# Alisah-Ozcan/GPU-NTT

Hardware: AMD Instinct MI355X
Metric: forward-NTTs/sec + achieved HBM GB/s, 64-bit Merge N=2^16 batch=1024 (higher is better)
Workload: dtype u64; 1 GPU; Merge-NTT Data64 log2N=16 batch=1024 forward (BASELINE configs[1]); log2N=16, batch_per_gpu=1024, reduction_poly=X_N_minus, modulus=576460756061519873, in_place=True, api=dropin, parallelism=batch-shard x1

## Files before the change

### gpu-ntt_amd/csrc/launch.hpp

```cpp
#pragma once

#include <hip/hip_runtime.h>

#include <stdexcept>

#include "gpuntt/common/common.cuh"
#include "merge_kernels.hpp"

#ifndef GPUNTT_SHADOW_GRID
#define GPUNTT_SHADOW_GRID 512
#endif

namespace gpuntt
{
    namespace host
    {
        void note_launch(const char* kernel_expr, int family = -1);
    }
}
#define GPUNTT_LAUNCH(kernel, ...)                                                                                       \
    do                                                                                                                   \
    {                                                                                                                    \
        ::gpuntt::host::note_launch(#kernel);                                                                            \
        hipLaunchKernelGGL(kernel, __VA_ARGS__);                                                                         \
    } while (0)
#define GPUNTT_LAUNCH_FAMILY(family, kernel, ...)                                                                        \
    do                                                                                                                   \
    {                                                                                                                    \
        ::gpuntt::host::note_launch(#kernel, family);                                                                    \
        hipLaunchKernelGGL(kernel, __VA_ARGS__);                                                                         \
    } while (0)

namespace gpuntt
{
    namespace host
    {
        struct Pass
        {
            bool contig;
            int k;
            int p_lo;
            int in_b = 0;
            bool p4 = false;
        };

        struct Plan
        {
            Pass pass[8];
            int count;
        };

        inline Plan make_plan(int n, int contig_k = kern::TL)
        {
            Plan pl{};
            pl.count = 0;
            if (n <= kern::TL)
            {
                pl.pass[pl.count++] = Pass{true, n, 0};
                return pl;
            }
            if (contig_k > kern::TL)
                contig_k = kern::TL;
            if (contig_k < 8)
                contig_k = 8;
            const int s = n - contig_k;
            const int np = (s + 7) / 8;
            int top = n;
            for (int i = 0; i < np; i++)
            {
                const int k = s / np + ((i < s % np) ? 1 : 0);
                top -= k;
                pl.pass[pl.count++] = Pass{false, k, top};
            }
            pl.pass[pl.count++] = Pass{true, contig_k, 0};
            return pl;
// ... 39 lines not shown
```

### gpu-ntt_amd/csrc/lazy.hpp

```cpp
#pragma once

#include <hip/hip_runtime.h>

#include <cstdint>

namespace gpuntt
{
    namespace lazy
    {
        template <typename T> struct Tw;
        template <> struct alignas(16) Tw<uint64_t>
        {
            uint64_t w;
            uint64_t wp;
        };
        template <> struct alignas(8) Tw<uint32_t>
        {
            uint32_t w;
            uint32_t wp;
        };
        using Tw64 = Tw<uint64_t>;
        using Tw32 = Tw<uint32_t>;

        __device__ __forceinline__ uint32_t lo32(uint64_t v) { return static_cast<uint32_t>(v); }
// ... 51 lines not shown
            uint64_t d, cy;
            if constexpr (SB)
                asm("v_mad_u64_u32 %0, %1, %2, %3, -1" : "=v"(d), "=s"(cy) : "v"(a), "s"(b));
            else
                asm("v_mad_u64_u32 %0, %1, %2, %3, -1" : "=v"(d), "=s"(cy) : "v"(a), "v"(b));
            return d;
        }
        __device__ __forceinline__ uint32_t xad_not(uint32_t w, uint32_t u) { return (w ^ 0xffffffffu) + u; }

        template <int LIM, bool VQ = false> struct Mod64
        {
            static constexpr int TB = (LIM == 4) ? 2 : 4;
            static constexpr int LIMIT = LIM;
            static constexpr int MAX_BIT = (LIM == 16 || LIM == 31) ? 60 : (LIM == 8 ? 61 : 62);
            uint64_t q;
            uint64_t qneg;
            NormConst nc;
            uint32_t zero;
            uint32_t one;

            __device__ __forceinline__ void set(uint64_t modulus, const NormConst& n)
            {
                q = modulus;
                qneg = 0 - modulus;
                nc = n;
                asm("v_mov_b32 %0, 0" : "=v"(zero));
                asm("v_mov_b32 %0, 1" : "=v"(one));
            }
            template <bool HI = false> __device__ __forceinline__ uint64_t reduce_2q(uint64_t x) const
            {
                const uint32_t xt = HI ? hi32(x) : static_cast<uint32_t>(x >> nc.sh);
                const uint32_t k = __umulhi(xt, nc.M) >> nc.c;
                const uint64_t r = static_cast<uint64_t>(k) * lo32(qneg) + x;
                return r + (static_cast<uint64_t>(k * hi32(qneg)) << 32);
            }
            __device__ __forceinline__ uint64_t kq(int k) const { return q * static_cast<uint64_t>(k); }
            __device__ __forceinline__ bool hi_norm() const { return nc.hi != 0u; }

            template <bool UNI, bool ZERO = false>
            __device__ __forceinline__ uint64_t mul_acc(uint64_t x, const Tw64& t, uint64_t acc) const
            {
                if constexpr (LIM == 4)
                {
                    const uint64_t p = csub<2>(mul_acc_raw<UNI, true>(x, t, 0));
                    return ZERO ? p : acc + p;
                }
                else
                    return mul_acc_raw<UNI, ZERO>(x, t, acc);
            }
            template <bool UNI, bool ZERO>
            __device__ __forceinline__ uint64_t mul_acc_raw(uint64_t x, const Tw64& t, uint64_t acc) const
            {
                const uint32_t x0 = lo32(x), x1 = hi32(x);
                const uint32_t h2 = __umulhi(x0, hi32(t.wp));
                uint64_t qh, carry;
                if constexpr (UNI)
                    asm("v_mul_hi_u32 v126, %2, %3\n\tv_mad_u64_u32 %0, %1, %2, %4, v[126:127]"
                        : "=v"(qh), "=s"(carry)
                        : "v"(x1), "s"(lo32(t.wp)), "s"(hi32(t.wp)), "{v127}"(zero)
                        : "v126");
                else
                    asm("v_mul_hi_u32 v126, %2, %3\n\tv_mad_u64_u32 %0, %1, %2, %4, v[126:127]"
                        : "=v"(qh), "=s"(carry)
                        : "v"(x1), "v"(lo32(t.wp)), "v"(hi32(t.wp)), "{v127}"(zero)
                        : "v126");
                qh = static_cast<uint64_t>(h2) * one + qh;
                uint64_t c = static_cast<uint64_t>(x0) * hi32(t.w);
// ... 145 lines not shown
            if constexpr (B > 2)
                x = m.template csub<2>(x);
            if constexpr (B > 1)
                x = m.template csub<1>(x);
            return x;
        }

        constexpr int ceil_pow2(int v)
        {
            int p = 1;
            while (p < v)
                p <<= 1;
            return p;
        }
        constexpr int csub_k(int b) { return ceil_pow2(b) / 2; }

        struct CtPlan
        {
            int ku;
            int out;
        };
        constexpr CtPlan ct_plan(int bu, int limit, int tb)
        {
            CtPlan p{0, 0};
            if (bu + tb > limit)
            {
                p.ku = csub_k(bu);
                bu = p.ku;
            }
            p.out = bu + tb;
            return p;
        }

        struct GsPlan
        {
            int ku, kv;
            int c;
            int ko;
            int out_u;
        };
        constexpr GsPlan gs_plan(int bu, int bv, int limit)
        {
            GsPlan p{0, 0, 0, 0, 0};
            const int half = limit / 2;
            if (bu > half)
            {
                p.ku = csub_k(bu);
                bu = p.ku;
            }
            if (bv > half)
            {
                p.kv = csub_k(bv);
                bv = p.kv;
            }
            p.c = ceil_pow2(bv);
            int out = bu + bv;
            if (out > half)
            {
                p.ko = csub_k(out);
                out = p.ko;
            }
            p.out_u = out;
            return p;
        }
    }
}
// ... 1 lines not shown
```

### gpu-ntt_amd/csrc/lazy_launch.hpp

```cpp
#pragma once

#include <hip/hip_runtime.h>

#include <string>

#include "launch.hpp"
#include "merge_lazy_kernels.hpp"

namespace gpuntt
{
    namespace host
    {
        constexpr int LAZY_MAX_N_POWER = 28;

        constexpr int lazy_u32_tile_override() { return 0; }
        constexpr int lazy_u64_big_tiles() { return 14; }

        bool lazy_two_sweep_big();
        bool lazy_contig_p4();
        void note_contig_p4_launch();
        unsigned long long contig_p4_launches();
        constexpr int LAZY_P4_N_POWER = 16;
        constexpr unsigned long long lazy_u32_small_batch() { return 0x7fffffffull; }
        template <typename T> inline int lazy_tile_log(int n, bool inverse = false, unsigned long long polys = 0)
// ... 320 lines not shown
        extern template void launch_pass_lazy_lim<false, 4>(const Pass&, bool, bool, const kern::LazyArgsT<uint64_t>&, hipStream_t);
        template <bool INV, int LIMSEL>
        void launch_fourstep_lim(int what, int log_n1, const kern::LazyArgsT<uint64_t>& a, hipStream_t stream);
        extern template void launch_fourstep_lim<false, 8>(int, int, const kern::LazyArgsT<uint64_t>&, hipStream_t);
        extern template void launch_fourstep_lim<true, 8>(int, int, const kern::LazyArgsT<uint64_t>&, hipStream_t);
        extern template void launch_fourstep_lim<false, 4>(int, int, const kern::LazyArgsT<uint64_t>&, hipStream_t);
        extern template void launch_fourstep_lim<true, 4>(int, int, const kern::LazyArgsT<uint64_t>&, hipStream_t);
        template <typename TU> inline bool modulus_fast(const Modulus<TU>& m)
        {
            const TU max_bit = (sizeof(TU) == 8) ? TU(62) : TU(lazy::Mod<TU>::MAX_BIT);
            return m.value >= 3 && m.bit <= max_bit;
        }
        template <typename TU> inline int modulus_lim(const Modulus<TU>& m)
        {
            if (sizeof(TU) != 8)
                return 0;
            return m.bit == TU(62) ? 4 : (m.bit == TU(61) ? 8 : 0);
        }
        void launch_pass_lazy31(const Pass& p, int tile_log, bool in_first, bool last, const kern::LazyArgsT<uint64_t>& a,
                                hipStream_t stream);
        constexpr bool lazy_lim31_enabled() { return true; }
        constexpr unsigned lazy_order_flags() { return 0u; }
        template <bool INV>
        void launch_pass_lazy_u32w(const Pass& p, int tile_log, bool in_first, bool last,
                                   const kern::LazyArgsT<uint32_t>& a, hipStream_t stream);
        template <>
        void launch_pass_lazy_u32w<false>(const Pass&, int, bool, bool, const kern::LazyArgsT<uint32_t>&, hipStream_t);
        template <>
        void launch_pass_lazy_u32w<true>(const Pass&, int, bool, bool, const kern::LazyArgsT<uint32_t>&, hipStream_t);
        inline bool lazy_wide_modulus32(uint32_t q) { return q >= 3 && q < (1u << 29); }
        inline bool lazy_lim31_modulus(uint64_t q) { return q >= 3 && q <= 0xffffffffffffffffull / 31; }
        extern template void launch_pass_lazy_lim<true, 4>(const Pass&, bool, bool, const kern::LazyArgsT<uint64_t>&, hipStream_t);

        inline int fwd_bound_after(int bound, int k, int limit, int tb)
        {
            for (int s = 0; s < k; s++)
                bound = lazy::ct_plan(bound, limit, tb).out;
            return bound;
        }

        template <typename T, bool INV>
        inline void run_transform_lazy(kern::LazyArgsT<T> base, unsigned first_in_flags,
                                       unsigned last_out_flags, hipStream_t stream, int forced_tl = 0, int low_stages = 0)
        {
            const int tl = (sizeof(T) == 8 && base.lim && base.lim != 31)
                               ? 12
                               : (forced_tl ? forced_tl : lazy_tile_log_merge<T>(base.n, INV, base.total >> base.n));
            const int pn = (!INV && low_stages > 0) ? low_stages : base.n;
            const bool partial = pn != base.n;
            if constexpr (sizeof(T) == 4)
                if (!partial && base.n == tl && tl >= 12 && tl <= 15 &&
                    (tl == 15 || ((lazy_e32_mask() >> tl) & 1u) != 0u) && (base.total & ((1ull << tl) - 1ull)) == 0ull)
                {
                    kern::LazyArgsT<uint32_t> a = base;
                    a.p_lo = 0;
                    a.flags |= first_in_flags | last_out_flags;
                    return launch_ring_e32<INV>(tl, base.lim, a, stream);
                }
            if (base.mods != nullptr && base.mod_count > 1 && base.n < tl && base.n - kern::R < 6)
            {
                if (base.n < LAZY_MIN_RNS_N_POWER || partial)
                    throw std::invalid_argument("internal: RNS ring too small for the fast path");
                kern::LazyArgsT<T> a = base;
                a.p_lo = 0;
                a.flags |= first_in_flags | last_out_flags;
                return launch_small_rns_lazy<T, INV>(base.n, a, stream);
            }
            const bool big2 = sizeof(T) == 8 && tl == 14 && pn >= 23 && !partial;
            const Plan pl = make_plan_tl(pn, tl, tl == 12 ? (partial ? lazy_contig_k(pn) : lazy_contig_k_merge<T>(pn, INV)) : tl,
                                         big2 ? 10 : (sizeof(T) == 4 && tl == 15) ? 9 : 8);
            const void* src = base.in;
            int fwd_bound = partial ? 16 : 1;
            for (int i = 0; i < pl.count; i++)
            {
                Pass p = INV ? pl.pass[pl.count - 1 - i] : pl.pass[i];
                if (!INV && sizeof(T) == 8 && base.lim == 31)
                {
                    p.in_b = fwd_bound;
                    fwd_bound = fwd_bound_after(fwd_bound, p.k, 31, 4);
                }
                kern::LazyArgsT<T> a = base;
                a.in = src;
                a.p_lo = p.p_lo;
                a.flags |= lazy_order_flags();
                const bool first = (i == 0) && !partial;
                if (i == 0)
                    a.flags |= first_in_flags;
                if (i == pl.count - 1)
                    a.flags |= last_out_flags;
                if (((pl.count - 1 - i) & 1) != 0 && lazy_reverse_passes())
                    a.flags |= kern::F_REVERSE;
                const int tlp = (sizeof(T) == 8 && !p.contig && p.k <= 8) ? 12 : (sizeof(T) == 4 && tl == 15 && !p.contig) ? 14 : tl;
                const unsigned long long polys = base.total >> base.n;
                a.batch = (p.contig && base.n >= 20 && base.n >= tlp && polys >= 2 && polys <= 0x7fffffffull &&
                           (polys << base.n) == base.total)
                              ? static_cast<int>(polys)
                              : 0;
                if constexpr (sizeof(T) == 8 && !INV)
                {
                    const unsigned long long mc = base.mods != nullptr ? static_cast<unsigned long long>(base.mod_count) : 1ull;
                    p.p4 = p.contig && p.k == 10 && tlp == 12 && i == pl.count - 1 && pl.count > 1 && !partial &&
                           base.n == LAZY_P4_N_POWER && base.poly_shift == base.n && mc >= 1 && polys % (4ull * mc) == 0 &&
                           (polys << base.n) == base.total && base.poly_order == nullptr && base.mod_order == nullptr &&
                           base.mul_in == nullptr && a.batch == 0 && lazy_contig_p4();
                }
                if constexpr (sizeof(T) == 4)
                {
                    const bool edge = INV ? (i == 0 && pl.count > 1) : (i == pl.count - 1 && (pl.count > 1 || partial));
                    if (p.contig && p.k == tlp && (tlp == 12 || tlp == 14 || tlp == 15) && edge &&
                        (tlp == 15 || ((lazy_e32_mask() >> 16) & 1u) != 0u))
                    {
                        launch_tile_e32<INV>(tlp, base.lim, a, stream);
                        src = base.out;
                        continue;
                    }
                }
                if constexpr (sizeof(T) == 8)
                {
                    if (base.lim == 8)
                        launch_pass_lazy_lim<INV, 8>(p, first, i == pl.count - 1, a, stream);
                    else if (base.lim == 4)
                        launch_pass_lazy_lim<INV, 4>(p, first, i == pl.count - 1, a, stream);
                    else if (base.lim == 31)
                    {
                        if constexpr (!INV)
// ... 20 lines not shown
```

### gpu-ntt_amd/csrc/lazy_launch_impl.hpp

```cpp
#pragma once

#include "lazy_launch.hpp"

namespace gpuntt
{
    namespace host
    {
        template <typename T, int TLOG, bool INV, bool CONTIG, int K, int IN_BOUND, bool LAST, int LIMSEL = 0, bool P4 = false>
        inline void launch_lazy_one(const kern::LazyArgsT<T>& a, unsigned grid, hipStream_t stream)
        {
            if constexpr (P4)
                note_contig_p4_launch();
            GPUNTT_LAUNCH_FAMILY(LIMSEL, (kern::merge_pass_lazy<T, TLOG, INV, CONTIG, K, IN_BOUND, LAST, LIMSEL, 0, P4>), dim3(grid),
                               dim3(kern::LTile<TLOG>::NT), 0, stream, a);
            GPUNTT_HIP_CHECK(hipGetLastError());
        }

        template <typename T, int TLOG, bool INV, int LIMSEL = 0>
        void dispatch_tl(const Pass& p, bool in_first, bool last, const kern::LazyArgsT<T>& a,
                         hipStream_t stream)
        {
            constexpr int LIM = lazy::Mod<T, LIMSEL>::LIMIT;
            constexpr int TILE = kern::LTile<TLOG>::TILE;
            const unsigned long long tiles = (a.total + TILE - 1) >> TLOG;
            if (tiles == 0)
                return;
            if (tiles > 0x7fffffffull)
                throw std::invalid_argument("batch_size * N too large for one launch");
            const unsigned grid = lazy_grid_cap<T, LIMSEL>(tiles, a.go_flag);
#define GPUNTT_ONE(CONTIG_, K_, IN_, LAST_)                                                      \
    return launch_lazy_one<T, TLOG, INV, CONTIG_, K_, IN_, LAST_, LIMSEL>(a, grid, stream)
            if constexpr (sizeof(T) == 8 && TLOG >= 13)
            {
                if (p.contig && p.k == TLOG)
                {
                    if (in_first && last)
                        GPUNTT_ONE(true, TLOG, 1, true);
                    if constexpr (!INV)
                    {
                        if (!in_first && last)
                            GPUNTT_ONE(true, TLOG, LIM, true);
                    }
                    else
                    {
                        if (in_first && !last)
                            GPUNTT_ONE(true, TLOG, 1, false);
                    }
                }
                if constexpr (TLOG == 14 && !INV)
                    if (!p.contig && in_first && !last)
                    {
                        if (p.k == 9)
                            GPUNTT_ONE(false, 9, 1, false);
                        if (p.k == 10)
                            GPUNTT_ONE(false, 10, 1, false);
                    }
                throw std::invalid_argument("internal: unsupported 64-bit big-tile pass");
            }
            else
            {
            if (p.contig)
            {
// ... 12 lines not shown
                            case 8: GPUNTT_ONE(true, 8, 1, true);
                            case 9: GPUNTT_ONE(true, 9, 1, true);
                            case 10: GPUNTT_ONE(true, 10, 1, true);
                            case 11: GPUNTT_ONE(true, 11, 1, true);
                            case 12: GPUNTT_ONE(true, 12, 1, true);
                            default: break;
                        }
                    else if constexpr (TLOG == 13)
                    {
                        if (p.k == 13)
                            GPUNTT_ONE(true, 13, 1, true);
                    }
                    else
                        switch (p.k)
                        {
                            case 13: GPUNTT_ONE(true, 13, 1, true);
                            case 14: GPUNTT_ONE(true, 14, 1, true);
                            default: break;
                        }
                }
                else if (!INV && !in_first && last)
                {
                    if constexpr (!INV)
                    {
                        if constexpr (TLOG == 12)
                            switch (p.k)
                            {
                                case 8: GPUNTT_ONE(true, 8, LIM, true);
                                case 9: GPUNTT_ONE(true, 9, LIM, true);
                                case 10:
                                    if constexpr (sizeof(T) == 8)
                                        if (p.p4)
                                        {
                                            if constexpr (LIM == 31)
                                                if (p.in_b > 0 && p.in_b <= 27)
                                                    return launch_lazy_one<T, TLOG, INV, true, 10, 27, true, LIMSEL, true>(a, grid, stream);
                                            return launch_lazy_one<T, TLOG, INV, true, 10, LIM, true, LIMSEL, true>(a, grid, stream);
                                        }
                                    if constexpr (LIM == 31)
                                        if (p.in_b > 0 && p.in_b <= 27)
                                            GPUNTT_ONE(true, 10, 27, true);
                                    GPUNTT_ONE(true, 10, LIM, true);
                                case 11: GPUNTT_ONE(true, 11, LIM, true);
                                case 12: GPUNTT_ONE(true, 12, LIM, true);
                                default: break;
                            }
                        else if constexpr (TLOG == 14)
                        {
                            if (p.k == 14)
                                GPUNTT_ONE(true, 14, LIM, true);
                            if (p.k == 13)
                                GPUNTT_ONE(true, 13, LIM, true);
                        }
                    }
                }
                else if (INV && in_first && !last)
                {
                    if constexpr (INV)
                    {
                        if constexpr (TLOG == 12)
                            switch (p.k)
                            {
                                case 8: GPUNTT_ONE(true, 8, 1, false);
                                case 9: GPUNTT_ONE(true, 9, 1, false);
                                case 10: GPUNTT_ONE(true, 10, 1, false);
                                case 11: GPUNTT_ONE(true, 11, 1, false);
                                case 12: GPUNTT_ONE(true, 12, 1, false);
                                default: break;
                            }
                        else if constexpr (TLOG == 14)
                            if (p.k == 14)
                                GPUNTT_ONE(true, 14, 1, false);
                    }
                }
                throw std::invalid_argument("internal: unsupported contiguous pass in the fast path");
            }
            if constexpr (TLOG == 12 || TLOG == 14)
            {
                if constexpr (!INV)
                {
                    if (!last)
                        switch (p.k * 2 + (in_first ? 1 : 0))
                        {
#define GPUNTT_CASE(KK)                                                                          \
    case KK * 2 + 1: GPUNTT_ONE(false, KK, 1, false);                                            \
    case KK * 2: GPUNTT_ONE(false, KK, LIM, false);
                            GPUNTT_CASE(1)
                            GPUNTT_CASE(2)
                            GPUNTT_CASE(3)
                            GPUNTT_CASE(4)
                            GPUNTT_CASE(5)
                            GPUNTT_CASE(6)
                            GPUNTT_CASE(7)
                            GPUNTT_CASE(8)
#undef GPUNTT_CASE
                            default: break;
                        }
                    if constexpr (sizeof(T) == 4 && TLOG == 14)
                        if (!last && in_first && p.k == 9)
                            GPUNTT_ONE(false, 9, 1, false);
                    if constexpr ((LIMSEL == 0 || (LIMSEL == 4 && sizeof(T) == 8)) && TLOG == 12)
                        if (last)
                            switch (p.k * 2 + (in_first ? 1 : 0))
                            {
#define GPUNTT_CASE(KK)                                                                          \
    case KK * 2 + 1: GPUNTT_ONE(false, KK, 1, true);                                             \
    case KK * 2: GPUNTT_ONE(false, KK, LIM, true);
                                GPUNTT_CASE(1)
                                GPUNTT_CASE(2)
                                GPUNTT_CASE(3)
                                GPUNTT_CASE(4)
                                GPUNTT_CASE(5)
                                GPUNTT_CASE(6)
// ... 316 lines not shown
```

### gpu-ntt_amd/csrc/merge_lazy_kernels.hpp

```cpp
#pragma once

#include "contig_p4_map.hpp"
#include "lazy.hpp"
#include "merge_kernels.hpp"

namespace gpuntt
{
    namespace kern
    {
        template <typename T> struct LazyArgsT
        {
            const void* in;
            T* out;
            const lazy::Tw<T>* tw;
            const Modulus<T>* mods;
            T q;
            T q_bit;
            T q_mu;
            const lazy::Tw<T>* ninv_arr;
            lazy::Tw<T> ninv;
            lazy::NormConst norm;
            const lazy::NormConst* norm_arr;
            const unsigned* go_flag;
            const int* mod_order;
// ... 63 lines not shown
                }
            }
            __device__ __forceinline__ LTileMap(int n, int pass_p_lo) : LTileMap(n, pass_p_lo, blockIdx.x) {}
            __device__ __forceinline__ unsigned long long flat(int e) const
            {
                return base + part(static_cast<unsigned>(e));
            }
            __device__ __forceinline__ int gpos(int p) const
            {
                constexpr int L = LGeo<TLOG, CONTIG, K>::L;
                if constexpr (CONTIG)
                    return p;
                else
                    return p_lo + (p - L);
            }
            __device__ __forceinline__ void remap_poly(const int* order, int n)
            {
                const unsigned long long poly = base >> n;
                base = (static_cast<unsigned long long>(static_cast<unsigned>(order[poly])) << n) |
                       (base & ((1ull << n) - 1));
            }
            __device__ __forceinline__ unsigned part(unsigned e) const
            {
                constexpr int L = LGeo<TLOG, CONTIG, K>::L;
                if constexpr (CONTIG && SEG)
                    return ((e >> K) << p_lo) | (e & ((1u << K) - 1u));
                else if constexpr (CONTIG)
                    return e;
                else
                    return ((e >> L) << p_lo) | (e & ((1u << L) - 1u));
            }
        };

        template <int TLOG, bool INV, bool CONTIG, int K, int IN_BOUND, int LIMIT, int TB, int SKIP = 0> struct PassSched
        {
            using G = LGeo<TLOG, CONTIG, K>;
            static_assert(SKIP == 0 || (INV && CONTIG && SKIP < K), "partial passes: inverse, contiguous");
            static constexpr int TL = TLOG;
            static constexpr int NR = (K - SKIP + R - 1) / R;
            struct Data
            {
                int ku[NR][R][EPT / 2];
                int kv[NR][R][EPT / 2];
                int c[NR][R][EPT / 2];
                int ko[NR][R][EPT / 2];
                int bout[NR][EPT];
                int bin[NR];
                int final_bound;
            };
            static constexpr int SHORT = (K - SKIP) - R * (NR - 1);
            static constexpr int stages_of(int r)
            {
                return INV ? ((r == NR - 1) ? SHORT : R) : ((r == 0) ? SHORT : R);
            }
            static constexpr int first_pos(int r)
            {
                if (INV)
                    return G::L + SKIP + r * R;
                return (r == 0) ? (G::L + K - 1) : (G::L + K - 1 - SHORT - (r - 1) * R);
            }
            static constexpr int wl_of(int r)
            {
                int w = INV ? (first_pos(r) + stages_of(r) - R) : (first_pos(r) - R + 1);
                const int lo = CONTIG ? 0 : (G::L > TL - R ? TL - R : G::L);
                return w < lo ? lo : (w > TL - R ? TL - R : w);
            }
            static constexpr Data make()
            {
                Data d{};
                int bound_in = IN_BOUND;
                for (int r = 0; r < NR; r++)
                {
                    int b[EPT] = {};
                    for (int j = 0; j < EPT; j++)
                        b[j] = bound_in;
                    d.bin[r] = bound_in;
                    for (int s = 0; s < stages_of(r); s++)
                    {
                        const int p = INV ? (first_pos(r) + s) : (first_pos(r) - s);
                        const int jb = p - wl_of(r);
                        for (int h = 0; h < EPT / 2; h++)
                        {
                            const int j0 = (h & ((1 << jb) - 1)) | ((h >> jb) << (jb + 1));
                            const int j1 = j0 | (1 << jb);
                            if (!INV)
                            {
                                const lazy::CtPlan pl = lazy::ct_plan(b[j0], LIMIT, TB);
                                d.ku[r][s][h] = pl.ku;
                                b[j0] = b[j1] = pl.out;
                            }
                            else
                            {
                                const lazy::GsPlan pl = lazy::gs_plan(b[j0], b[j1], LIMIT);
                                d.ku[r][s][h] = pl.ku;
                                d.kv[r][s][h] = pl.kv;
                                d.c[r][s][h] = pl.c;
                                d.ko[r][s][h] = pl.ko;
                                b[j0] = pl.out_u;
                                b[j1] = TB;
                            }
                        }
                    }
                    int mx = 0;
                    for (int j = 0; j < EPT; j++)
                    {
                        d.bout[r][j] = b[j];
                        mx = b[j] > mx ? b[j] : mx;
                    }
                    bound_in = mx;
                }
                d.final_bound = bound_in;
                return d;
            }
            static constexpr Data d = make();
            static_assert(d.final_bound <= LIMIT, "lazy bound exceeds the headroom");
            static_assert(!INV || d.final_bound <= LIMIT / 2, "an inverse pass must hand over values below LIMIT / 2");
        };

        template <int TLOG, typename T = uint32_t> struct LOcc
        {
            static constexpr int WAVES = (TLOG >= 14 && sizeof(T) == 4) ? 8 : 4;
        };

        constexpr int TW_PER_ROUND = EPT - 1;

        template <bool NT_, typename T> __device__ __forceinline__ T ld_stream(const T* p)
        {
            if constexpr (NT_)
                return __builtin_nontemporal_load(p);
            else
                return *p;
        }
        template <bool NT_, typename T> __device__ __forceinline__ void st_stream(T* p, T v)
        {
            if constexpr (NT_)
                __builtin_nontemporal_store(v, p);
            else
                *p = v;
        }

        __device__ __forceinline__ void wave_sync()
        {
            __builtin_amdgcn_fence(__ATOMIC_RELEASE, "wavefront");
            __builtin_amdgcn_wave_barrier();
            __builtin_amdgcn_fence(__ATOMIC_ACQUIRE, "wavefront");
        }

        constexpr int XP_L1 = 5;
        template <int K> __device__ __forceinline__ unsigned xp_swap_fwd(unsigned f)
        {
// ... 27 lines not shown
            for (int j = 0; j < N; j++)
            {
                if constexpr (sizeof(T) == 8)
                    asm volatile("" : "+v"(v[j])::"memory");
                else
                    asm volatile("" : "+v"(v[j])::"memory");
            }
        }

        enum class Fst : int
        {
            none = 0,
            nat_rows = 2,
            inv_first = 3
        };
        enum class Xp : int
        {
            none = 0,
            small_fwd = 1,
            small_inv = 2,
            small_nat_fwd = 3,
            small_nat_inv = 4,
            first_gather = 5
        };

        template <typename T, int N> __device__ __forceinline__ void relayout_barrier(T (&loaded)[N])
        {
            pin_loaded(loaded);
            __syncthreads();
        }

        template <typename T, int TLOG, bool INV, bool CONTIG, int K, int IN_BOUND, bool LAST,
                  Fst FST = Fst::none, int LIM = 0, Xp XP = Xp::none, int SKIP = 0, bool VQ = false, int ROWLEN = 0,
                  bool P4 = false>
        __device__ __forceinline__ void pass_body(const LazyArgsT<T>& a, T* lds, T q_value, T q_bit, T q_mu,
                                                  int mi, unsigned long long fst_poly = 0,
                                                  unsigned fst_tile = 0, long long blk_override = -1,
                                                  unsigned fst_seg = 0)
        {
            using G = LGeo<TLOG, CONTIG, K>;
            using M = lazy::Mod<T, LIM, VQ>;
            using SCH = PassSched<TLOG, INV, CONTIG, K, IN_BOUND, M::LIMIT, M::TB, SKIP>;
            using TW = lazy::Tw<T>;
            static_assert(!VQ || (FST == Fst::none && XP == Xp::none && SKIP == 0), "per-lane moduli: plain passes");
            static_assert(!(VQ && CONTIG) || (K >= R && K < TLOG && IN_BOUND == 1 && LAST),
                          "per-lane moduli, contiguous: single-pass transforms of rings of 16 .. tile/2 coefficients");
            static_assert(!P4 || (sizeof(T) == 8 && TLOG == p4::TLOG && !INV && CONTIG && K == p4::K && IN_BOUND != 1 && LAST &&
                                  FST == Fst::none && XP == Xp::none && SKIP == 0 && !VQ),
                          "four-polynomial tile: the forward 64-bit 10-stage last pass");
            constexpr bool HAS_FST = (FST != Fst::none);
            constexpr int TL = TLOG;
            constexpr int NT = LTile<TLOG>::NT;
            constexpr int NR_ = SCH::NR;
            static_assert(!P4 || (SCH::NR == p4::ROUNDS && SCH::wl_of(0) == p4::window(0) && SCH::wl_of(1) == p4::window(1) &&
                                  SCH::wl_of(P4 ? 2 : 0) == p4::window(2) && SCH::stages_of(0) == 2 && SCH::stages_of(1) == 4 &&
                                  SCH::stages_of(P4 ? 2 : 0) == 4 && SCH::first_pos(0) == 9 && SCH::first_pos(1) == 7 &&
                                  SCH::first_pos(P4 ? 2 : 0) == 3),
                          "contig_p4_map.hpp assumes this round schedule");

            constexpr bool MULTI_POLY = CONTIG && (K < TL) && (IN_BOUND == 1) && (LAST || HAS_FST);
            constexpr bool WIO_OK = CONTIG && (!HAS_FST || FST == Fst::inv_first) && !MULTI_POLY && (TL >= 10);
            constexpr int WIO = 6;
            const int t = threadIdx.x;
            constexpr bool SEG = (FST == Fst::nat_rows);
            using Map = LTileMap<TLOG, CONTIG, K, SEG>;
            Map map = P4    ? Map(fst_poly)
                      : SEG ? Map((fst_poly << a.poly_shift) +
                                      ((static_cast<unsigned long long>(fst_tile) << (TL - K)) << a.row_log) +
                                      (static_cast<unsigned long long>(fst_seg) << K),
                                  a.row_log)
                      : HAS_FST ? Map((fst_poly << a.poly_shift) + (static_cast<unsigned long long>(fst_tile) << TL))
                            : Map(a.n, a.p_lo,
                                  blk_override >= 0 ? static_cast<unsigned long long>(blk_override)
                                                    : static_cast<unsigned long long>(blockIdx.x));
            const bool tile_in_range = (CONTIG && !HAS_FST && !P4) ? ((map.base + LTile<TLOG>::TILE) <= a.total) : true;
// ... 337 lines not shown
                        __syncthreads();
                        const T* lw = lds + lds_pad(elem_of<WL>(t, 0));
#pragma unroll
                        for (int j = 0; j < EPT; j++)
                            v[j] = lw[lds_joff<WL>(j)];
                    }
                }
                else
                {
                    const T* lw = lds + (P4 ? static_cast<int>(p4::lds_slot(p4::elem(r, static_cast<unsigned>(t), 0)))
                                            : lds_pad(elem_of<WL>(t, 0)));
#pragma unroll
                    for (int j = 0; j < EPT; j++)
                        v[j] = lw[lds_joff<WL>(j)];
                }

                TW tw_cur[TW_PER_ROUND];
                if constexpr (TW_AHEAD)
                {
#pragma unroll
                    for (int i = 0; i < TW_PER_ROUND; i++)
                        tw_cur[i] = tw_next[i];
                }
                else
                {
                    load_twiddles(r_, tw_cur);
                }

                int off = 0;
                static_for<STAGES>([&](auto s_) {
                    constexpr int s = decltype(s_)::value;
                    constexpr int p = INV ? (FIRST_POS + s) : (FIRST_POS - s);
                    constexpr int jb = p - WL;
                    static_for<EPT / 2>([&](auto h_) {
                        constexpr int h = decltype(h_)::value;
                        constexpr int j0 = (h & ((1 << jb) - 1)) | ((h >> jb) << (jb + 1));
                        constexpr int j1 = j0 | (1 << jb);
                        constexpr int kk = j0 >> (jb + 1);
                        const TW tw = tw_cur[off + kk];
                        constexpr bool UNI_TW = UNIFORM_R && !VQ;
                        if constexpr (!INV)
                        {
                            constexpr int ku = SCH::d.ku[r][s][h];
                            T U = v[j0];
                            if constexpr (ku != 0)
                                U = m.template csub<ku>(U);
                            bool unit = false;
                            if constexpr (UNI_TW && r == 0 && s == 0 && IN_BOUND <= M::TB && !HAS_FST)
                                unit = (tw.w == 1);
                            {
                                const T nu = unit ? static_cast<T>(U + v[j1]) : m.template mul_acc<UNI_TW>(v[j1], tw, U);
                                v[j0] = nu;
                                v[j1] = static_cast<T>(m.shl1_add(U, m.kq(M::TB)) - nu);
                            }
                        }
                        else
                        {
                            constexpr int ku = SCH::d.ku[r][s][h];
                            constexpr int kv = SCH::d.kv[r][s][h];
                            constexpr int c = SCH::d.c[r][s][h];
                            T U = v[j0], V = v[j1];
                            if constexpr (ku != 0)
                                U = m.template csub<ku>(U);
                            if constexpr (kv != 0)
                                V = m.template csub<kv>(V);
                            if constexpr (LAST && r == NR_ - 1 && s == STAGES - 1)
                                v[j0] = m.template mul<!VQ>(U + V, ninv);
                            else
                            {
                                constexpr int ko = SCH::d.ko[r][s][h];
                                T S = U + V;
                                if constexpr (ko != 0)
                                    S = m.template csub<ko>(S);
                                v[j0] = S;
                            }
                            v[j1] = m.template mul<UNI_TW>(U + m.kq(c) - V, tw);
                        }
                    });
// ... 378 lines not shown
        }
        template <typename T, int TLOG, bool INV>
        __device__ __forceinline__ void fourstep_tile_generic(const LazyArgsT<T>& a, T* lds, unsigned long long poly,
                                                              const dev::ModCtx<T>& m, T ninv)
        {
            constexpr int NT = LTile<TLOG>::NT, N = 1 << TLOG, L1 = XP_L1, L2 = TLOG - XP_L1;
            static_assert(N == NT * EPT, "16 coefficients per thread");
            const int t = threadIdx.x;
            const T* in = static_cast<const T*>(a.in) + (poly << TLOG);
            T* out = a.out + (poly << TLOG);
            for (int e = t; e < N; e += NT)
                lds[e] = in[e];
            __syncthreads();
            fs_stages<T, INV, NT>(lds, N, a.fs_n1, L1, m);
            T tmp[EPT];
#pragma unroll
            for (int k = 0; k < EPT; k++)
            {
                const unsigned o = static_cast<unsigned>(t + NT * k);
                const unsigned i = o >> L2, r = o & ((1u << L2) - 1u);
                tmp[k] = m.mul(lds[(r << L1) | i], a.fs_w[o]);
            }
            __syncthreads();
#pragma unroll
            for (int k = 0; k < EPT; k++)
                lds[t + NT * k] = tmp[k];
            __syncthreads();
            fs_stages<T, INV, NT>(lds, N, a.fs_n2, L2, m);
            for (int e = t; e < N; e += NT)
                out[e] = INV ? m.mul(lds[e], ninv) : lds[e];
        }

        template <typename T, int TLOG, bool INV, bool CONTIG, int K, int IN_BOUND, bool LAST, int LIM = 0, int SKIP = 0,
                  bool P4 = false>
        __global__ __launch_bounds__(LTile<TLOG>::NT, (LOcc<TLOG, T>::WAVES)) void merge_pass_lazy(LazyArgsT<T> a)
        {
            using M = lazy::Mod<T, LIM>;
            constexpr int SK = INV ? SKIP : 0;
            using SCH = PassSched<TLOG, INV, CONTIG, K, IN_BOUND, M::LIMIT, M::TB, SK>;
            constexpr bool NEEDS_LDS = (SCH::NR > 1) || (SCH::wl_of(0) < 4);
            __shared__ T lds[P4 ? p4::LDS_ELEMS : (NEEDS_LDS ? LTile<TLOG>::LDS_ELEMS : 1)];

            if constexpr (SKIP != 0 && TLOG == 12 && CONTIG)
                if (self_fallback_call<T, LIM>(a))
                {
                    if constexpr (INV)
                        fs_phase2_chunk<T, true, LTile<12>::NT>(a, blockIdx.x, a.n, fs_modulus(a), fs_ninv(a));
                    else
                        fs_phase2_chunk<T, false, LTile<12>::NT>(a, blockIdx.x, a.n - a.n2_log, fs_modulus(a), T(0));
                    return;
                }
            if (not_my_call<T, LIM>(a.go_flag, a.flags))
                return;
            for_each_block<WalksTiles<T, LIM>::value>(
                static_cast<unsigned>((a.total + LTile<TLOG>::TILE - 1) >> TLOG), [&](unsigned bidx, unsigned nblk) {
            T qv = a.q, qb = a.q_bit, qm = a.q_mu;
            int mi = 0;
            const unsigned bx = (a.flags & F_REVERSE) ? (nblk - 1u - bidx) : bidx;
            if constexpr (P4)
            {
                const unsigned mc = (a.mods != nullptr) ? static_cast<unsigned>(a.mod_count) : 1u;
                const int seg_log = a.n - K;
                const unsigned seg = uniform32(bx & ((1u << seg_log) - 1u));
                const unsigned pm = bx >> seg_log;
                mi = static_cast<int>(uniform32(pm % mc));
                const unsigned long long poly0 = static_cast<unsigned long long>(pm / mc) * (4u * mc) + static_cast<unsigned>(mi);
                if (a.mods != nullptr)
                {
                    const Modulus<T> md = a.mods[mi];
                    qv = md.value;
                    qb = md.bit;
                    qm = md.mu;
                }
                pass_body<T, TLOG, INV, CONTIG, K, IN_BOUND, LAST, Fst::none, LIM, Xp::none, SK, false, 0, true>(
                    a, lds, qv, qb, qm, mi, uniform64((poly0 << a.n) + (static_cast<unsigned long long>(seg) << K)), seg);
                return;
            }
            long long blk = static_cast<long long>(bx);
            if (a.batch > 1)
            {
                unsigned poly, tile;
                poly_minor_order(bx, static_cast<unsigned>(a.batch), a.n - TLOG, poly, tile, a.flags);
                blk = static_cast<long long>(
                    uniform64((static_cast<unsigned long long>(poly) << (a.n - TLOG)) | tile));
            }
            if (a.mods != nullptr)
            {
                const LTileMap<TLOG, CONTIG, K> map(a.n, a.p_lo, static_cast<unsigned long long>(blk));
                unsigned long long poly = map.flat(0) >> a.poly_shift;
                if constexpr (CONTIG && K < TLOG && K - R >= 6 && IN_BOUND == 1 && LAST)
                    poly += threadIdx.x >> (K - R);
                mi = static_cast<int>(uniform32(static_cast<unsigned>(poly % static_cast<unsigned>(a.mod_count))));
                const Modulus<T> md = a.mods[a.mod_order != nullptr ? a.mod_order[mi] : mi];
                qv = md.value;
                qb = md.bit;
                qm = md.mu;
            }
            pass_body<T, TLOG, INV, CONTIG, K, IN_BOUND, LAST, Fst::none, LIM, Xp::none, SK>(a, lds, qv, qb, qm, mi, 0, 0, blk);
                });
        }

        template <typename T> struct VqLim
        {
            static constexpr int LIM = (sizeof(T) == 8) ? 4 : 0;
        };
        template <typename T, bool INV, int K, int IN_BOUND, bool LAST>
        __global__ __launch_bounds__(LTile<12>::NT, (LOcc<12, T>::WAVES)) void merge_pass_lazy_vq(LazyArgsT<T> a)
        {
            constexpr int LIM = VqLim<T>::LIM;
            using M = lazy::Mod<T, LIM, true>;
            using SCH = PassSched<12, INV, false, K, IN_BOUND, M::LIMIT, M::TB, 0>;
            constexpr bool NEEDS_LDS = (SCH::NR > 1) || (SCH::wl_of(0) < 4);
            __shared__ T lds[NEEDS_LDS ? LTile<12>::LDS_ELEMS : 1];
            if (a.go_flag != nullptr && *a.go_flag == GO_GENERIC)
                return;
            pass_body<T, 12, INV, false, K, IN_BOUND, LAST, Fst::none, LIM, Xp::none, 0, true>(a, lds, 0, 0, 0, 0, 0, 0,
                                                                                       static_cast<long long>(blockIdx.x));
        }

        template <typename T, bool INV, int K, int LIM>
        __global__ __launch_bounds__(LTile<12>::NT, (LOcc<12, T>::WAVES)) void merge_pass_lazy_vqc(LazyArgsT<T> a)
        {
            __shared__ T lds[LTile<12>::LDS_ELEMS];
            if (a.go_flag != nullptr)
            {
                const unsigned mine = sizeof(T) != 8 ? GO_LAZY
                                      : (LIM == 4 ? GO_LAZY_4Q : (LIM == 8 ? GO_LAZY_8Q : (a.lim == 31 ? GO_LAZY_31Q : GO_LAZY)));
                if (*a.go_flag != mine)
                    return;
            }
            for_each_block<WalksTiles<T, LIM>::value>(
// ... 150 lines not shown
```

Before: 2.543 million NTT/s.

## Plan lazy-reduction bounds per whole forward pass with DP and hand-off caps

Replaces the greedy per-stage lazy conditional-subtraction plan for forward 64-bit passes with a compile-time dynamic-programming search. The search picks, for each butterfly stage, between no reduction, a conditional subtract, or a cheaper Barrett-style estimate reduction. It also caps the bound handed from the first strided pass to the final contiguous pass, so the successor can be compiled for a tighter input bound. In addition, the high-word add in reduce_2q is rewritten as an explicit 32-bit add. This is meant to cut modular-reduction ALU work in the merge NTT, at the cost of more template instantiations and more complex host-side bound planning.

```diff
diff --git a/gpu-ntt_amd/csrc/launch.hpp b/gpu-ntt_amd/csrc/launch.hpp
--- a/gpu-ntt_amd/csrc/launch.hpp
+++ b/gpu-ntt_amd/csrc/launch.hpp
@@ -41,6 +41,7 @@
             int k;
             int p_lo;
             int in_b = 0;
+            int cap = 0;
             bool p4 = false;
         };
 
diff --git a/gpu-ntt_amd/csrc/lazy.hpp b/gpu-ntt_amd/csrc/lazy.hpp
--- a/gpu-ntt_amd/csrc/lazy.hpp
+++ b/gpu-ntt_amd/csrc/lazy.hpp
@@ -107,7 +107,10 @@
                 const uint32_t xt = HI ? hi32(x) : static_cast<uint32_t>(x >> nc.sh);
                 const uint32_t k = __umulhi(xt, nc.M) >> nc.c;
                 const uint64_t r = static_cast<uint64_t>(k) * lo32(qneg) + x;
-                return r + (static_cast<uint64_t>(k * hi32(qneg)) << 32);
+                const uint32_t kh = k * hi32(qneg);
+                uint32_t h;
+                asm("v_add_u32 %0, %1, %2" : "=v"(h) : "v"(hi32(r)), "v"(kh));
+                return (static_cast<uint64_t>(h) << 32) | lo32(r);
             }
             __device__ __forceinline__ uint64_t kq(int k) const { return q * static_cast<uint64_t>(k); }
             __device__ __forceinline__ bool hi_norm() const { return nc.hi != 0u; }
@@ -319,6 +322,109 @@
             return p;
         }
 
+        constexpr int CT_MAX_STAGES = 16;
+        constexpr int CT_MAX_BOUND = 32;
+        constexpr int CT_COST_CSUB = 4;
+        constexpr int CT_COST_EST = 5;
+        constexpr int CT_EST = -1;
+        struct CtSched
+        {
+            int ku[CT_MAX_STAGES];
+            int bu[CT_MAX_STAGES];
+            int out;
+            int cost;
+            bool ok;
+        };
+        constexpr CtSched ct_sched_plain(int bound, int k, int limit, int tb)
+        {
+            CtSched s{};
+            for (int i = 0; i < k; i++)
+            {
+                const CtPlan p = ct_plan(bound, limit, tb);
+                s.ku[i] = p.ku;
+                s.bu[i] = bound;
+                s.cost += p.ku != 0 ? CT_COST_CSUB : 0;
+                bound = p.out;
+            }
+            s.out = bound;
+            s.ok = bound <= limit;
+            return s;
+        }
+        constexpr CtSched ct_search(int bound, int k, int limit, int tb, int cap, int price_csub, int price_est)
+        {
+            constexpr int INF = 1 << 20;
+            CtSched s{};
+            if (k > CT_MAX_STAGES || limit >= CT_MAX_BOUND || bound > limit || bound < 1)
+                return s;
+            int cost[CT_MAX_STAGES + 1][CT_MAX_BOUND] = {};
+            int from[CT_MAX_STAGES + 1][CT_MAX_BOUND] = {};
+            int how[CT_MAX_STAGES + 1][CT_MAX_BOUND] = {};
+            for (int i = 0; i <= k; i++)
+                for (int b = 0; b < CT_MAX_BOUND; b++)
+                    cost[i][b] = INF;
+            cost[0][bound] = 0;
+            for (int i = 0; i < k; i++)
+                for (int b = 1; b <= limit; b++)
+                {
+                    if (cost[i][b] >= INF)
+                        continue;
+                    const int kh = (b + 1) / 2;
+                    const int nb[3] = {b, kh, 2};
+                    const int ku[3] = {0, kh, CT_EST};
+                    const int pr[3] = {0, price_csub, price_est};
+                    for (int c = 0; c < 3; c++)
+                    {
+                        if (c == 1 && kh >= b)
+                            continue;
+                        if (c == 2 && b <= 2)
+                            continue;
+                        const int o = nb[c] + tb;
+                        if (o > limit)
+                            continue;
+                        const int t = cost[i][b] + pr[c];
+                        if (t < cost[i + 1][o])
+                        {
+                            cost[i + 1][o] = t;
+                            from[i + 1][o] = b;
+                            how[i + 1][o] = ku[c];
+                        }
+                    }
+                }
+            int best = -1;
+            for (int b = 1; b <= limit && b <= cap; b++)
+                if (cost[k][b] < INF && (best < 0 || cost[k][b] < cost[k][best]))
+                    best = b;
+            if (best < 0)
+                return s;
+            s.out = best;
+            s.cost = cost[k][best];
+            s.ok = true;
+            for (int i = k, b = best; i > 0; i--)
+            {
+                s.ku[i - 1] = how[i][b];
+                s.bu[i - 1] = from[i][b];
+                b = from[i][b];
+            }
+            return s;
+        }
+        constexpr CtSched ct_sched(int bound, int k, int limit, int tb, int cap)
+        {
+            const CtSched plain = ct_sched_plain(bound, k, limit, tb);
+            const CtSched best = ct_search(bound, k, limit, tb, cap, CT_COST_CSUB, CT_COST_EST);
+            if (plain.ok && plain.out <= cap && (!best.ok || plain.cost <= best.cost))
+                return plain;
+            return best;
+        }
+        constexpr int ct_handoff_cap(int k_next, int limit, int tb)
+        {
+            const int base = ct_search(2 + tb, k_next, limit, tb, limit, 1, 1).cost;
+            int cap = 2 + tb;
+            for (int b = 2 + tb; b <= limit; b++)
+                if (ct_search(b, k_next, limit, tb, limit, 1, 1).cost == base)
+                    cap = b;
+            return cap;
+        }
+
         struct GsPlan
         {
             int ku, kv;
diff --git a/gpu-ntt_amd/csrc/lazy_launch.hpp b/gpu-ntt_amd/csrc/lazy_launch.hpp
--- a/gpu-ntt_amd/csrc/lazy_launch.hpp
+++ b/gpu-ntt_amd/csrc/lazy_launch.hpp
@@ -376,10 +376,84 @@
         inline bool lazy_lim31_modulus(uint64_t q) { return q >= 3 && q <= 0xffffffffffffffffull / 31; }
         extern template void launch_pass_lazy_lim<true, 4>(const Pass&, bool, bool, const kern::LazyArgsT<uint64_t>&, hipStream_t);
 
-        inline int fwd_bound_after(int bound, int k, int limit, int tb)
-        {
-            for (int s = 0; s < k; s++)
-                bound = lazy::ct_plan(bound, limit, tb).out;
+        constexpr int FWD_CAP_CONTIG_K = 10;
+        constexpr bool fwd_cap_strided_k(int k) { return k == 4 || k == 6; }
+        struct FwdOutRow
+        {
+            int out[lazy::CT_MAX_STAGES + 1];
+        };
+        constexpr FwdOutRow fwd_out_row(int bound, int limit, int cap)
+        {
+            FwdOutRow r{};
+            for (int k = 1; k <= lazy::CT_MAX_STAGES; k++)
+            {
+                const lazy::CtSched s = lazy::ct_sched(bound, k, limit, 4, cap);
+                r.out[k] = s.ok ? s.out : 0;
+            }
+            return r;
+        }
+        template <int LIMIT> struct FwdBounds
+        {
+            static constexpr int CAP10 = lazy::ct_handoff_cap(FWD_CAP_CONTIG_K, LIMIT, 4);
+            static constexpr FwdOutRow from_1 = fwd_out_row(1, LIMIT, LIMIT);
+            static constexpr FwdOutRow from_1_capped = fwd_out_row(1, LIMIT, CAP10);
+            static constexpr FwdOutRow from_cap = fwd_out_row(CAP10, LIMIT, LIMIT);
+            static constexpr FwdOutRow from_limit = fwd_out_row(LIMIT, LIMIT, LIMIT);
+            static int after(int bound, int k, int cap)
+            {
+                if (k < 1 || k > lazy::CT_MAX_STAGES)
+                    return 0;
+                if (cap == CAP10 && bound == 1)
+                    return from_1_capped.out[k];
+                if (cap != 0)
+                    return 0;
+                return bound == 1 ? from_1.out[k] : bound == CAP10 ? from_cap.out[k] : bound == LIMIT ? from_limit.out[k] : 0;
+            }
+        };
+        inline int fwd_handoff_cap10(int limit) { return limit == 31 ? FwdBounds<31>::CAP10 : FwdBounds<16>::CAP10; }
+        inline int fwd_bound_after(int bound, int k, int limit, int cap = 0)
+        {
+            const int out = limit == 31 ? FwdBounds<31>::after(bound, k, cap) : limit == 16 ? FwdBounds<16>::after(bound, k, cap) : 0;
+            if (out == 0)
+                throw std::invalid_argument("internal: no range plan for a forward pass");
+            return out;
+        }
+        inline int fwd_pass_cap(const Plan& pl, int i, int tile_log, bool first, int limit)
+        {
+            if (pl.count != 2 || i != 0 || !first || tile_log != 12)
+                return 0;
+            const Pass& p = pl.pass[0];
+            const Pass& nx = pl.pass[1];
+            if (p.contig || !fwd_cap_strided_k(p.k) || !nx.contig || nx.k != FWD_CAP_CONTIG_K)
+                return 0;
+            return fwd_handoff_cap10(limit);
+        }
+        inline int fwd_inst_bound(const Pass& p, int tile_log, bool in_first, bool last, int limit)
+        {
+            if (in_first)
+                return 1;
+            if (p.contig && last && tile_log == 12 && p.k == FWD_CAP_CONTIG_K && p.in_b > 0)
+            {
+                const int cap = fwd_handoff_cap10(limit);
+                if (p.in_b <= cap)
+                    return cap;
+            }
+            return limit;
+        }
+
+        inline int fwd_pass_tile64(const Pass& p, int tl) { return (!p.contig && p.k <= 8) ? 12 : tl; }
+        inline int fwd_plan_bounds(Plan& pl, int tl, bool partial, int limit)
+        {
+            int bound = partial ? 16 : 1;
+            for (int i = 0; i < pl.count; i++)
+            {
+                Pass& p = pl.pass[i];
+                const int tlp = fwd_pass_tile64(p, tl);
+                const bool first = i == 0 && !partial;
+                p.in_b = bound;
+                p.cap = fwd_pass_cap(pl, i, tlp, first, limit);
+                bound = fwd_bound_after(fwd_inst_bound(p, tlp, first, i == pl.count - 1, limit), p.k, limit, p.cap);
+            }
             return bound;
         }
 
@@ -411,18 +485,15 @@
                 return launch_small_rns_lazy<T, INV>(base.n, a, stream);
             }
             const bool big2 = sizeof(T) == 8 && tl == 14 && pn >= 23 && !partial;
-            const Plan pl = make_plan_tl(pn, tl, tl == 12 ? (partial ? lazy_contig_k(pn) : lazy_contig_k_merge<T>(pn, INV)) : tl,
+            Plan pl = make_plan_tl(pn, tl, tl == 12 ? (partial ? lazy_contig_k(pn) : lazy_contig_k_merge<T>(pn, INV)) : tl,
                                          big2 ? 10 : (sizeof(T) == 4 && tl == 15) ? 9 : 8);
             const void* src = base.in;
-            int fwd_bound = partial ? 16 : 1;
+            if (!INV && sizeof(T) == 8 && (base.lim == 31 || base.lim == 0))
+                fwd_plan_bounds(pl, tl, partial, base.lim == 31 ? 31 : 16);
             for (int i = 0; i < pl.count; i++)
             {
                 Pass p = INV ? pl.pass[pl.count - 1 - i] : pl.pass[i];
-                if (!INV && sizeof(T) == 8 && base.lim == 31)
-                {
-                    p.in_b = fwd_bound;
-                    fwd_bound = fwd_bound_after(fwd_bound, p.k, 31, 4);
-                }
+                const int tlp = sizeof(T) == 8 ? fwd_pass_tile64(p, tl) : (tl == 15 && !p.contig) ? 14 : tl;
                 kern::LazyArgsT<T> a = base;
                 a.in = src;
                 a.p_lo = p.p_lo;
@@ -434,7 +505,6 @@
                     a.flags |= last_out_flags;
                 if (((pl.count - 1 - i) & 1) != 0 && lazy_reverse_passes())
                     a.flags |= kern::F_REVERSE;
-                const int tlp = (sizeof(T) == 8 && !p.contig && p.k <= 8) ? 12 : (sizeof(T) == 4 && tl == 15 && !p.contig) ? 14 : tl;
                 const unsigned long long polys = base.total >> base.n;
                 a.batch = (p.contig && base.n >= 20 && base.n >= tlp && polys >= 2 && polys <= 0x7fffffffull &&
                            (polys << base.n) == base.total)
diff --git a/gpu-ntt_amd/csrc/lazy_launch_impl.hpp b/gpu-ntt_amd/csrc/lazy_launch_impl.hpp
--- a/gpu-ntt_amd/csrc/lazy_launch_impl.hpp
+++ b/gpu-ntt_amd/csrc/lazy_launch_impl.hpp
@@ -6,12 +6,13 @@
 {
     namespace host
     {
-        template <typename T, int TLOG, bool INV, bool CONTIG, int K, int IN_BOUND, bool LAST, int LIMSEL = 0, bool P4 = false>
+        template <typename T, int TLOG, bool INV, bool CONTIG, int K, int IN_BOUND, bool LAST, int LIMSEL = 0, bool P4 = false,
+                  int CAP = 0>
         inline void launch_lazy_one(const kern::LazyArgsT<T>& a, unsigned grid, hipStream_t stream)
         {
             if constexpr (P4)
                 note_contig_p4_launch();
-            GPUNTT_LAUNCH_FAMILY(LIMSEL, (kern::merge_pass_lazy<T, TLOG, INV, CONTIG, K, IN_BOUND, LAST, LIMSEL, 0, P4>), dim3(grid),
+            GPUNTT_LAUNCH_FAMILY(LIMSEL, (kern::merge_pass_lazy<T, TLOG, INV, CONTIG, K, IN_BOUND, LAST, LIMSEL, 0, P4, CAP>), dim3(grid),
                                dim3(kern::LTile<TLOG>::NT), 0, stream, a);
             GPUNTT_HIP_CHECK(hipGetLastError());
         }
@@ -28,6 +29,10 @@
             if (tiles > 0x7fffffffull)
                 throw std::invalid_argument("batch_size * N too large for one launch");
             const unsigned grid = lazy_grid_cap<T, LIMSEL>(tiles, a.go_flag);
+            constexpr bool CAPPED = sizeof(T) == 8 && !INV && TLOG == 12 && (LIM == 16 || LIM == 31);
+            constexpr int CAP10 = CAPPED ? FwdBounds<CAPPED ? LIM : 16>::CAP10 : LIM;
+            if (!CAPPED && p.cap != 0)
+                throw std::invalid_argument("internal: no capped hand-off in this kernel family");
 #define GPUNTT_ONE(CONTIG_, K_, IN_, LAST_)                                                      \
     return launch_lazy_one<T, TLOG, INV, CONTIG_, K_, IN_, LAST_, LIMSEL>(a, grid, stream)
             if constexpr (sizeof(T) == 8 && TLOG >= 13)
@@ -106,14 +111,14 @@
                                     if constexpr (sizeof(T) == 8)
                                         if (p.p4)
                                         {
-                                            if constexpr (LIM == 31)
-                                                if (p.in_b > 0 && p.in_b <= 27)
-                                                    return launch_lazy_one<T, TLOG, INV, true, 10, 27, true, LIMSEL, true>(a, grid, stream);
+                                            if constexpr (CAPPED)
+                                                if (fwd_inst_bound(p, TLOG, in_first, last, LIM) == CAP10)
+                                                    return launch_lazy_one<T, TLOG, INV, true, 10, CAP10, true, LIMSEL, true>(a, grid, stream);
                                             return launch_lazy_one<T, TLOG, INV, true, 10, LIM, true, LIMSEL, true>(a, grid, stream);
                                         }
-                                    if constexpr (LIM == 31)
-                                        if (p.in_b > 0 && p.in_b <= 27)
-                                            GPUNTT_ONE(true, 10, 27, true);
+                                    if constexpr (CAPPED)
+                                        if (fwd_inst_bound(p, TLOG, in_first, last, LIM) == CAP10)
+                                            GPUNTT_ONE(true, 10, CAP10, true);
                                     GPUNTT_ONE(true, 10, LIM, true);
                                 case 11: GPUNTT_ONE(true, 11, LIM, true);
                                 case 12: GPUNTT_ONE(true, 12, LIM, true);
@@ -153,6 +158,18 @@
             {
                 if constexpr (!INV)
                 {
+                    if constexpr (CAPPED)
+                        if (p.cap != 0)
+                        {
+                            if (!last && in_first && p.cap == CAP10)
+                                switch (p.k)
+                                {
+                                    case 4: return launch_lazy_one<T, TLOG, INV, false, 4, 1, false, LIMSEL, false, CAP10>(a, grid, stream);
+                                    case 6: return launch_lazy_one<T, TLOG, INV, false, 6, 1, false, LIMSEL, false, CAP10>(a, grid, stream);
+                                    default: break;
+                                }
+                            throw std::invalid_argument("internal: unsupported capped strided pass in the fast path");
+                        }
                     if (!last)
                         switch (p.k * 2 + (in_first ? 1 : 0))
                         {
diff --git a/gpu-ntt_amd/csrc/merge_lazy_kernels.hpp b/gpu-ntt_amd/csrc/merge_lazy_kernels.hpp
--- a/gpu-ntt_amd/csrc/merge_lazy_kernels.hpp
+++ b/gpu-ntt_amd/csrc/merge_lazy_kernels.hpp
@@ -119,10 +119,15 @@
             }
         };
 
-        template <int TLOG, bool INV, bool CONTIG, int K, int IN_BOUND, int LIMIT, int TB, int SKIP = 0> struct PassSched
+        template <int TLOG, bool INV, bool CONTIG, int K, int IN_BOUND, int LIMIT, int TB, int SKIP = 0, int CAP = 0,
+                  bool EST = false>
+        struct PassSched
         {
             using G = LGeo<TLOG, CONTIG, K>;
             static_assert(SKIP == 0 || (INV && CONTIG && SKIP < K), "partial passes: inverse, contiguous");
+            static_assert(!EST || (!INV && SKIP == 0 && K <= lazy::CT_MAX_STAGES), "whole-pass plans: forward passes");
+            static_assert(CAP == 0 || EST, "a hand-off cap needs the whole-pass plan");
+            static constexpr int HANDOFF_CAP = CAP == 0 ? LIMIT : CAP;
             static constexpr int TL = TLOG;
             static constexpr int NR = (K - SKIP + R - 1) / R;
             struct Data
@@ -156,6 +161,8 @@
             {
                 Data d{};
                 int bound_in = IN_BOUND;
+                const lazy::CtSched whole = EST ? lazy::ct_sched(IN_BOUND, K, LIMIT, TB, HANDOFF_CAP) : lazy::CtSched{};
+                int g = 0;
                 for (int r = 0; r < NR; r++)
                 {
                     int b[EPT] = {};
@@ -170,7 +177,13 @@
                         {
                             const int j0 = (h & ((1 << jb) - 1)) | ((h >> jb) << (jb + 1));
                             const int j1 = j0 | (1 << jb);
-                            if (!INV)
+                            if (!INV && EST)
+                            {
+                                const int ku = whole.ku[g];
+                                d.ku[r][s][h] = ku;
+                                b[j0] = b[j1] = (ku == lazy::CT_EST ? 2 : (ku > 0 ? ku : b[j0])) + TB;
+                            }
+                            else if (!INV)
                             {
                                 const lazy::CtPlan pl = lazy::ct_plan(b[j0], LIMIT, TB);
                                 d.ku[r][s][h] = pl.ku;
@@ -187,6 +200,7 @@
                                 b[j1] = TB;
                             }
                         }
+                        g++;
                     }
                     int mx = 0;
                     for (int j = 0; j < EPT; j++)
@@ -196,13 +210,19 @@
                     }
                     bound_in = mx;
                 }
-                d.final_bound = bound_in;
+                d.final_bound = (EST && (!whole.ok || whole.out != bound_in)) ? LIMIT + 1 : bound_in;
                 return d;
             }
             static constexpr Data d = make();
             static_assert(d.final_bound <= LIMIT, "lazy bound exceeds the headroom");
+            static_assert(d.final_bound <= HANDOFF_CAP, "the pass hands over more than its successor was compiled for");
             static_assert(!INV || d.final_bound <= LIMIT / 2, "an inverse pass must hand over values below LIMIT / 2");
         };
+
+        template <typename T, bool INV, bool VQ, bool PLAIN> constexpr bool plans_whole_pass(int limit)
+        {
+            return !INV && sizeof(T) == 8 && !VQ && PLAIN && (limit == 16 || limit == 31);
+        }
 
         template <int TLOG, typename T = uint32_t> struct LOcc
         {
@@ -296,7 +316,7 @@
 
         template <typename T, int TLOG, bool INV, bool CONTIG, int K, int IN_BOUND, bool LAST,
                   Fst FST = Fst::none, int LIM = 0, Xp XP = Xp::none, int SKIP = 0, bool VQ = false, int ROWLEN = 0,
-                  bool P4 = false>
+                  bool P4 = false, int CAP = 0>
         __device__ __forceinline__ void pass_body(const LazyArgsT<T>& a, T* lds, T q_value, T q_bit, T q_mu,
                                                   int mi, unsigned long long fst_poly = 0,
                                                   unsigned fst_tile = 0, long long blk_override = -1,
@@ -304,7 +324,9 @@
         {
             using G = LGeo<TLOG, CONTIG, K>;
             using M = lazy::Mod<T, LIM, VQ>;
-            using SCH = PassSched<TLOG, INV, CONTIG, K, IN_BOUND, M::LIMIT, M::TB, SKIP>;
+            constexpr bool EST = plans_whole_pass<T, INV, VQ, (FST == Fst::none && XP == Xp::none)>(M::LIMIT);
+            static_assert(CAP == 0 || EST, "hand-off caps: plain forward 64-bit passes");
+            using SCH = PassSched<TLOG, INV, CONTIG, K, IN_BOUND, M::LIMIT, M::TB, SKIP, CAP, EST>;
             using TW = lazy::Tw<T>;
             static_assert(!VQ || (FST == Fst::none && XP == Xp::none && SKIP == 0), "per-lane moduli: plain passes");
             static_assert(!(VQ && CONTIG) || (K >= R && K < TLOG && IN_BOUND == 1 && LAST),
@@ -708,6 +730,21 @@
                     constexpr int s = decltype(s_)::value;
                     constexpr int p = INV ? (FIRST_POS + s) : (FIRST_POS - s);
                     constexpr int jb = p - WL;
+                    if constexpr (!INV && SCH::d.ku[r][s][0] == lazy::CT_EST)
+                    {
+                        if (m.hi_norm())
+                            static_for<EPT / 2>([&](auto h_) {
+                                constexpr int h = decltype(h_)::value;
+                                constexpr int j0 = (h & ((1 << jb) - 1)) | ((h >> jb) << (jb + 1));
+                                v[j0] = m.template reduce_2q<true>(v[j0]);
+                            });
+                        else
+                            static_for<EPT / 2>([&](auto h_) {
+                                constexpr int h = decltype(h_)::value;
+                                constexpr int j0 = (h & ((1 << jb) - 1)) | ((h >> jb) << (jb + 1));
+                                v[j0] = m.template reduce_2q<false>(v[j0]);
+                            });
+                    }
                     static_for<EPT / 2>([&](auto h_) {
                         constexpr int h = decltype(h_)::value;
                         constexpr int j0 = (h & ((1 << jb) - 1)) | ((h >> jb) << (jb + 1));
@@ -719,7 +756,7 @@
                         {
                             constexpr int ku = SCH::d.ku[r][s][h];
                             T U = v[j0];
-                            if constexpr (ku != 0)
+                            if constexpr (ku > 0)
                                 U = m.template csub<ku>(U);
                             bool unit = false;
                             if constexpr (UNI_TW && r == 0 && s == 0 && IN_BOUND <= M::TB && !HAS_FST)
@@ -1164,7 +1201,7 @@
         }
 
         template <typename T, int TLOG, bool INV, bool CONTIG, int K, int IN_BOUND, bool LAST, int LIM = 0, int SKIP = 0,
-                  bool P4 = false>
+                  bool P4 = false, int CAP = 0>
         __global__ __launch_bounds__(LTile<TLOG>::NT, (LOcc<TLOG, T>::WAVES)) void merge_pass_lazy(LazyArgsT<T> a)
         {
             using M = lazy::Mod<T, LIM>;
@@ -1204,7 +1241,7 @@
                     qb = md.bit;
                     qm = md.mu;
                 }
-                pass_body<T, TLOG, INV, CONTIG, K, IN_BOUND, LAST, Fst::none, LIM, Xp::none, SK, false, 0, true>(
+                pass_body<T, TLOG, INV, CONTIG, K, IN_BOUND, LAST, Fst::none, LIM, Xp::none, SK, false, 0, true, CAP>(
                     a, lds, qv, qb, qm, mi, uniform64((poly0 << a.n) + (static_cast<unsigned long long>(seg) << K)), seg);
                 return;
             }
@@ -1228,7 +1265,8 @@
                 qb = md.bit;
                 qm = md.mu;
             }
-            pass_body<T, TLOG, INV, CONTIG, K, IN_BOUND, LAST, Fst::none, LIM, Xp::none, SK>(a, lds, qv, qb, qm, mi, 0, 0, blk);
+            pass_body<T, TLOG, INV, CONTIG, K, IN_BOUND, LAST, Fst::none, LIM, Xp::none, SK, false, 0, false, CAP>(a, lds, qv, qb,
+                                                                                                                   qm, mi, 0, 0, blk);
                 });
         }
 
```

Result: faster. 2.585 million NTT/s, median of 6 (+1.6%).
